# ByteDance-Seed/VeOmni

Hardware: AMD Instinct MI355X
Metric: tokens/sec/node (higher is better)
Workload: dtype bf16; 1 GPU; qwen3-moe-30b FSDP2 bf16 seq4096; model=qwen3-moe-30b, global_batch=8, seq_len=4096, parallelism=dp1

## Files before the change

### include/veomni_hip.h

```cpp
#ifndef VEOMNI_HIP_H
#define VEOMNI_HIP_H

#include <stdint.h>

#ifdef __cplusplus
extern "C" {
#endif

const char* vh_last_error(void);

const char* vh_build_info(void);


int vh_expert_histogram(const int64_t* expert_index, int64_t n,
                        int num_experts, int32_t* out, void* stream);

int vh_moe_scatter_bf16(const uint16_t* x, const int32_t* index, uint16_t* out,
                        int64_t M, int64_t N, int topk, void* stream);

int vh_moe_gather_bf16(const uint16_t* x, const int32_t* index, uint16_t* out,
                       int64_t M, int64_t N, int topk, void* stream);


int vh_group_gemm_nk_bf16(const uint16_t* A, const uint16_t* B, uint16_t* C,
                          const int64_t* cumsum, int G, int64_t N, int64_t K,
                          int64_t total_rows, int trans_b, int accumulate,
                          int activation, void* stream);


int vh_group_gemm_nk8_bf16(const uint16_t* A, const uint16_t* B, uint16_t* C,
                           const int64_t* cumsum, int G, int64_t N, int64_t K,
                           int64_t total_rows, int trans_b, void* stream);

int vh_group_gemm_nk256s_bf16(const uint16_t* A, const uint16_t* B,
                              uint16_t* C, const int64_t* cumsum, int G,
                              int64_t N, int64_t K, int64_t total_rows,
                              void* stream);

int vh_group_gemm_mn8_bf16(const uint16_t* A, const uint16_t* B, uint16_t* C,
                           const int64_t* cumsum, int G, int64_t M, int64_t N,
                           void* stream);

int vh_group_gemm_mn_bf16(const uint16_t* A, const uint16_t* B, uint16_t* C,
                          const int64_t* cumsum, int G, int64_t M, int64_t N,
                          void* stream);

int vh_wtranspose_bf16(const uint16_t* src, uint16_t* dst, int E, int64_t M,
                       int64_t N, void* stream);

int vh_transpose_pad_bf16(const uint16_t* src, uint16_t* dst,
                          const int64_t* cumsum, const int64_t* padded_cumsum,
                          int G, int64_t C, int64_t padded_total, void* stream);

int vh_group_gemm_wg256_bf16(const uint16_t* A, const uint16_t* B, uint16_t* C,
                             const int64_t* padded_cumsum, int G, int64_t M,
                             int64_t N, int64_t PR, void* stream);


int vh_moe_silu_mul_weighted_bf16(const uint16_t* fc1, const uint16_t* w_row,
                                  uint16_t* out, int64_t rows, int64_t I,
                                  int has_w, void* stream);

int vh_moe_silu_mul_weighted_bwd_bf16(const uint16_t* dy, const uint16_t* fc1,
                                      const uint16_t* w_row, uint16_t* dfc1,
                                      float* dw_row, int64_t rows, int64_t I,
                                      int has_w, void* stream);

int vh_moe_silu_mul_clamp_weighted_bf16(const uint16_t* fc1,
                                        const uint16_t* w_row, uint16_t* out,
                                        int64_t rows, int64_t I, int has_w,
                                        float limit, void* stream);

int vh_moe_silu_mul_clamp_weighted_bwd_bf16(const uint16_t* dy,
                                            const uint16_t* fc1,
                                            const uint16_t* w_row,
                                            uint16_t* dfc1, float* dw_row,
                                            int64_t rows, int64_t I, int has_w,
                                            float limit, void* stream);

// ... 71 lines not shown
```

### veomni_amd/csrc/vh_group_gemm.hip

```cpp

#include "vh_common.h"
#include "../../include/veomni_hip.h"

namespace {

constexpr int BM = 128, BN = 128, BK = 64;
constexpr int THREADS = 256;

using bf16frag = __attribute__((ext_vector_type(8))) __bf16;

__device__ __forceinline__ void glds16(const bf16_t* g, bf16_t* l) {
  __builtin_amdgcn_global_load_lds(
      (const __attribute__((address_space(1))) unsigned int*)g,
      (__attribute__((address_space(3))) unsigned int*)l, 16, 0, 0);
}

__device__ __forceinline__ int swz(int row, int colb) {
  return colb ^ ((((row >> 1) ^ (row >> 3)) & 7) << 4);
}

struct KStage {
  const bf16_t* src[4];
  int lds_base[4];

// ... 263 lines not shown

  const int col_in = lane & 15;
  const int row_base_in = (lane >> 4) * 4;
#pragma unroll
  for (int i = 0; i < 4; ++i)
#pragma unroll
    for (int j = 0; j < 4; ++j)
#pragma unroll
      for (int rr = 0; rr < 4; ++rr) {
        int64_t m = (int64_t)bm * BM + wr * 64 + i * 16 + row_base_in + rr;
        int64_t n = (int64_t)bn * BN + wc * 64 + j * 16 + col_in;
        if (m < M && n < N) Cg[m * N + n] = f2bf(acc[i][j][rr]);
      }
}

}

extern "C" int vh_group_gemm_nk_bf16(const uint16_t* A, const uint16_t* B,
                                     uint16_t* C, const int64_t* cumsum, int G,
                                     int64_t N, int64_t K, int64_t total_rows,
                                     int trans_b, int accumulate,
                                     int activation, void* stream) {
  hipStream_t s = reinterpret_cast<hipStream_t>(stream);
  if (!accumulate && activation == 0 && trans_b && K % 64 == 0 && N >= 256 &&
      total_rows >= (int64_t)G * 256 && G <= 4096) {
    return vh_group_gemm_nk256s_bf16(A, B, C, cumsum, G, N, K, total_rows,
                                     stream);
  }
  if (!accumulate && activation == 0 && !trans_b && K % 32 == 0 && K >= 1024 &&
      N >= 1024 && total_rows >= 16 * G * 16) {
    return vh_group_gemm_nk8_bf16(A, B, C, cumsum, G, N, K, total_rows, 0,
                                  stream);
  }
  VH_CHECK(K % BK == 0, "K %% 64 != 0 (K=%lld)", (long long)K);
  VH_CHECK(N % 16 == 0, "N %% 16 != 0 (N=%lld)", (long long)N);
  VH_CHECK(G >= 1, "G < 1");
  int tiles_m = (int)((total_rows + BM - 1) / BM);
  if (tiles_m < 1) tiles_m = 1;
  int tiles_n = (int)((N + BN - 1) / BN);
  dim3 grid(tiles_m * tiles_n, G);
  size_t lds = 65536;

#define VH_DISPATCH(TB, AC, ACT_)                                              \
  hipLaunchKernelGGL((k_group_gemm_nk<TB, AC, ACT_>), grid, dim3(THREADS),     \
                     lds, s, reinterpret_cast<const bf16_t*>(A),               \
                     reinterpret_cast<const bf16_t*>(B),                       \
                     reinterpret_cast<bf16_t*>(C), cumsum, G, N, K, tiles_m,   \
                     tiles_n)

  if (trans_b) {
// ... 33 lines not shown
```

### veomni_amd/csrc/vh_group_gemm8.hip

```cpp

#include "vh_common.h"

namespace {

constexpr int BM8 = 256, BN8 = 256, KSUB = 32;
constexpr int THREADS8 = 512;

using bf16frag = __attribute__((ext_vector_type(8))) __bf16;

__device__ __forceinline__ void glds16(const bf16_t* g, bf16_t* l) {
  __builtin_amdgcn_global_load_lds(
      (const __attribute__((address_space(1))) unsigned int*)g,
      (__attribute__((address_space(3))) unsigned int*)l, 16, 0, 0);
}

__device__ __forceinline__ int swz32(int row, int colb) {
  return colb ^ (((row >> 2) & 3) << 4);
}

__device__ __forceinline__ void raw_barrier() {
  asm volatile("" ::: "memory");
  __builtin_amdgcn_s_barrier();
  asm volatile("" ::: "memory");
}
// ... 414 lines not shown
      int o = base + lane * 16;
      int row = o >> 7;
      int colb = o & 127;
      src[i] = s + row_of(row) * ld_elems + (swz64(row, colb) >> 1);
      lds_base[i] = base;
    }
  }

  __device__ __forceinline__ void stage(bf16_t* tile, int64_t k0) const {
#pragma unroll
    for (int i = 0; i < 4; ++i) glds16(src[i] + k0, tile + (lds_base[i] >> 1));
  }
};

__device__ __forceinline__ bf16frag frag_read64(const bf16_t* tile, int row0,
                                                int ks, int lane) {
  int row = row0 + (lane & 15);
  int colb = (ks * 32 + ((lane >> 4) << 3)) * 2;
  int off_b = row * 128 + swz64(row, colb);
  return *reinterpret_cast<const bf16frag*>(
      reinterpret_cast<const char*>(tile) + off_b);
}


__global__ void k_gg_sched(const int64_t* __restrict__ cumsum, int G,
                           int tiles_n, int* __restrict__ ws) {
  if (threadIdx.x == 0 && blockIdx.x == 0) {
    int total = 0;
    int64_t prev = 0;
    for (int g = 0; g < G; ++g) {
      int64_t m = cumsum[g] - prev;
      prev = cumsum[g];
      ws[1 + g] = total;
      total += (int)((m + BM8 - 1) / BM8) * tiles_n;
    }
    ws[1 + G] = total;
    ws[0] = total;
  }
}

__global__ __launch_bounds__(THREADS8, 2) void k_group_gemm_nk256s(
    const bf16_t* __restrict__ A, const bf16_t* __restrict__ B,
    bf16_t* __restrict__ C, const int64_t* __restrict__ cumsum, int G,
    int64_t N, int64_t K, int tiles_n, const int* __restrict__ ws) {
  extern __shared__ __attribute__((aligned(16))) char smem[];
  bf16_t* sm = reinterpret_cast<bf16_t*>(smem);
  auto ta = [&](int buf) { return sm + buf * 32768; };
  auto tb = [&](int buf) { return sm + 16384 + buf * 32768; };

  const int tid = threadIdx.x;
  const int lane = tid & 63;
  const int wave = tid >> 6;
  const int wr = wave >> 2, wc = wave & 3;

  const int total_tiles = ws[0];
  const int X = blockIdx.x & 7;
  const int slot = blockIdx.x >> 3;
  const int L = (total_tiles + 7) / 8;
  const int t_end = min((X + 1) * L, total_tiles);
  const int nk = (int)(K / BK64);

  for (int t = X * L + slot; t < t_end; t += 32) {
    int lo = 0, hi = G - 1;
    while (lo < hi) {
      int mid = (lo + hi + 1) >> 1;
      if (ws[1 + mid] <= t) lo = mid;
      else hi = mid - 1;
    }
    const int gid = lo;
    const int local = t - ws[1 + gid];
    const int tiles_m_g = (ws[2 + gid] - ws[1 + gid]) / tiles_n;
    const int bm = local % tiles_m_g;
    const int bn = local / tiles_m_g;

    const int64_t row_start = (gid > 0) ? cumsum[gid - 1] : 0;
    const int64_t m_size = cumsum[gid] - row_start;
    const bf16_t* Ag = A + row_start * K;
    const bf16_t* Bg = B + (int64_t)gid * N * K;
    bf16_t* Cg = C + row_start * N;

    KStage64 sa, sb;
    sa.init(Ag, K, [&](int r) -> int64_t {
      int64_t gm = (int64_t)bm * BM8 + r;
      return gm % m_size;
    }, tid);
    sb.init(Bg, K, [&](int r) -> int64_t {
      int64_t gn = (int64_t)bn * BN8 + r;
      return gn % N;
    }, tid);

    f32x4 acc[8][4];
#pragma unroll
    for (int i = 0; i < 8; ++i)
#pragma unroll
      for (int j = 0; j < 4; ++j) acc[i][j] = {0.f, 0.f, 0.f, 0.f};

    sa.stage(ta(0), 0);
    sb.stage(tb(0), 0);
    __syncthreads();
    int cur = 0;
    for (int kt = 0; kt < nk; ++kt) {
      if (kt + 1 < nk) {
        sa.stage(ta(cur ^ 1), (int64_t)(kt + 1) * BK64);
        sb.stage(tb(cur ^ 1), (int64_t)(kt + 1) * BK64);
      }
#pragma unroll
      for (int ks = 0; ks < 2; ++ks) {
        bf16frag af[4], bfr[4];
#pragma unroll
        for (int j = 0; j < 4; ++j) bfr[j] = frag_read64(tb(cur), wc * 64 + j * 16, ks, lane);
#pragma unroll
        for (int i = 0; i < 4; ++i) af[i] = frag_read64(ta(cur), wr * 128 + i * 16, ks, lane);
        __builtin_amdgcn_s_setprio(1);
#pragma unroll
        for (int i = 0; i < 4; ++i)
#pragma unroll
          for (int j = 0; j < 4; ++j)
            acc[i][j] = __builtin_amdgcn_mfma_f32_16x16x32_bf16(af[i], bfr[j], acc[i][j], 0, 0, 0);
        __builtin_amdgcn_s_setprio(0);
#pragma unroll
        for (int i = 0; i < 4; ++i) af[i] = frag_read64(ta(cur), wr * 128 + 64 + i * 16, ks, lane);
        __builtin_amdgcn_s_setprio(1);
#pragma unroll
        for (int i = 0; i < 4; ++i)
#pragma unroll
          for (int j = 0; j < 4; ++j)
            acc[i + 4][j] = __builtin_amdgcn_mfma_f32_16x16x32_bf16(af[i], bfr[j], acc[i + 4][j], 0, 0, 0);
        __builtin_amdgcn_s_setprio(0);
      }
      __syncthreads();
      cur ^= 1;
    }

    const int col_in = lane & 15;
    const int row_base_in = (lane >> 4) * 4;
#pragma unroll
    for (int i = 0; i < 8; ++i)
#pragma unroll
      for (int j = 0; j < 4; ++j)
#pragma unroll
        for (int rr = 0; rr < 4; ++rr) {
          int64_t m = (int64_t)bm * BM8 + wr * 128 + (i & 3) * 16 + (i >> 2) * 64 +
                      row_base_in + rr;
          int64_t n = (int64_t)bn * BN8 + wc * 64 + j * 16 + col_in;
          if (m < m_size && n < N) Cg[m * N + n] = f2bf(acc[i][j][rr]);
        }
  }
}

}

static int* vh_gg_sched_ws = nullptr;
static constexpr int VH_GG_SCHED_MAX_G = 4096;

extern "C" int vh_group_gemm_nk256s_bf16(const uint16_t* A, const uint16_t* B,
                                         uint16_t* C, const int64_t* cumsum,
                                         int G, int64_t N, int64_t K,
                                         int64_t total_rows, void* stream) {
  hipStream_t s = reinterpret_cast<hipStream_t>(stream);
  VH_CHECK(K % BK64 == 0, "K %% 64 != 0");
  VH_CHECK(N % 16 == 0, "N %% 16 != 0");
  VH_CHECK(G <= VH_GG_SCHED_MAX_G, "G > %d", VH_GG_SCHED_MAX_G);
  if (vh_gg_sched_ws == nullptr) {
    VH_HIP(hipMalloc(&vh_gg_sched_ws, (VH_GG_SCHED_MAX_G + 2) * sizeof(int)));
  }
  int tiles_n = (int)((N + BN8 - 1) / BN8);
  hipLaunchKernelGGL(k_gg_sched, dim3(1), dim3(64), 0, s, cumsum, G, tiles_n,
                     vh_gg_sched_ws);
  VH_HIP(hipGetLastError());
  hipLaunchKernelGGL(k_group_gemm_nk256s, dim3(256), dim3(THREADS8), 131072, s,
                     reinterpret_cast<const bf16_t*>(A),
                     reinterpret_cast<const bf16_t*>(B),
                     reinterpret_cast<bf16_t*>(C), cumsum, G, N, K, tiles_n,
                     vh_gg_sched_ws);
  VH_HIP(hipGetLastError());
  return 0;
}


namespace {

__global__ void k_transpose_pad(const bf16_t* __restrict__ src,
                                bf16_t* __restrict__ dst,
                                const int64_t* __restrict__ cumsum,
                                const int64_t* __restrict__ padded_cumsum,
                                int G, int64_t C, int64_t padded_total) {
  __shared__ __attribute__((aligned(16))) bf16_t t2[64][72];

  int64_t chunk = blockIdx.x;
  int64_t col0 = (int64_t)blockIdx.y * 64;
  int64_t p0 = chunk * 64;
  int lo = 0, hi = G;
  while (lo < hi) {
    int mid = (lo + hi) >> 1;
    if (p0 >= padded_cumsum[mid]) lo = mid + 1; else hi = mid;
  }
  int g = lo;
  if (g >= G) return;
  int64_t pstart = (g > 0) ? padded_cumsum[g - 1] : 0;
  int64_t sstart = (g > 0) ? cumsum[g - 1] : 0;
  int64_t kcount = cumsum[g] - sstart;
  int64_t local0 = p0 - pstart;

  const int tid = threadIdx.x;
  for (int r = tid / 8; r < 64; r += 32) {
    int64_t lr = local0 + r;
    const int cpos = (tid % 8) * 8;
    bf16x8 v = {};
    if (lr < kcount && col0 + cpos < C) {
      v = *reinterpret_cast<const bf16x8*>(src + (sstart + lr) * C + col0 + cpos);
    }
    *reinterpret_cast<bf16x8*>(&t2[r][cpos]) = v;
  }
  __syncthreads();
  for (int c = tid / 8; c < 64; c += 32) {
    int rpos = (tid % 8) * 8;
    if (col0 + c < C) {
      bf16x8 v;
#pragma unroll
      for (int j = 0; j < 8; ++j) v.v[j] = t2[rpos + j][c];
      *reinterpret_cast<bf16x8*>(dst + (col0 + c) * padded_total + p0 + rpos) = v;
    }
  }
}

__global__ __launch_bounds__(THREADS8, 2) void k_group_gemm_wg256s(
    const bf16_t* __restrict__ A, const bf16_t* __restrict__ B,
    bf16_t* __restrict__ C, const int64_t* __restrict__ padded_cumsum, int G,
    int64_t M, int64_t N, int64_t PR, int tiles_m, int tiles_n) {
  extern __shared__ __attribute__((aligned(16))) char smem[];
  bf16_t* sm = reinterpret_cast<bf16_t*>(smem);
  auto ta = [&](int buf) { return sm + buf * 32768; };
  auto tb = [&](int buf) { return sm + 16384 + buf * 32768; };

  const int tid = threadIdx.x;
  const int lane = tid & 63;
  const int wave = tid >> 6;
  const int wr = wave >> 2, wc = wave & 3;

  const int tpg = tiles_m * tiles_n;
  const int total = G * tpg;
  const int X = blockIdx.x & 7;
  const int slot = blockIdx.x >> 3;
  const int L = (total + 7) / 8;
  const int t_end = min((X + 1) * L, total);

  for (int t = X * L + slot; t < t_end; t += 32) {
    const int gid = t / tpg;
    const int local = t - gid * tpg;
    const int bm = local % tiles_m;
    const int bn = local / tiles_m;

    const int64_t p_start = (gid > 0) ? padded_cumsum[gid - 1] : 0;
    const int64_t klen = padded_cumsum[gid] - p_start;
    bf16_t* Cg = C + (int64_t)gid * M * N;

    f32x4 acc[8][4];
#pragma unroll
    for (int i = 0; i < 8; ++i)
#pragma unroll
      for (int j = 0; j < 4; ++j) acc[i][j] = {0.f, 0.f, 0.f, 0.f};

    if (klen > 0) {
      const bf16_t* Ag = A + p_start;
      const bf16_t* Bg = B + p_start;
      KStage64 sa, sb;
      sa.init(Ag, PR, [&](int r) -> int64_t {
        int64_t gm = (int64_t)bm * BM8 + r;
        return gm % M;
      }, tid);
      sb.init(Bg, PR, [&](int r) -> int64_t {
        int64_t gn = (int64_t)bn * BN8 + r;
        return gn % N;
      }, tid);

      const int nk = (int)(klen / BK64);
      sa.stage(ta(0), 0);
      sb.stage(tb(0), 0);
      __syncthreads();
      int cur = 0;
      for (int kt = 0; kt < nk; ++kt) {
        if (kt + 1 < nk) {
          sa.stage(ta(cur ^ 1), (int64_t)(kt + 1) * BK64);
          sb.stage(tb(cur ^ 1), (int64_t)(kt + 1) * BK64);
        }
#pragma unroll
        for (int ks = 0; ks < 2; ++ks) {
          bf16frag af[4], bfr[4];
#pragma unroll
          for (int j = 0; j < 4; ++j) bfr[j] = frag_read64(tb(cur), wc * 64 + j * 16, ks, lane);
#pragma unroll
          for (int i = 0; i < 4; ++i) af[i] = frag_read64(ta(cur), wr * 128 + i * 16, ks, lane);
          __builtin_amdgcn_s_setprio(1);
#pragma unroll
          for (int i = 0; i < 4; ++i)
#pragma unroll
            for (int j = 0; j < 4; ++j)
              acc[i][j] = __builtin_amdgcn_mfma_f32_16x16x32_bf16(af[i], bfr[j], acc[i][j], 0, 0, 0);
          __builtin_amdgcn_s_setprio(0);
#pragma unroll
          for (int i = 0; i < 4; ++i) af[i] = frag_read64(ta(cur), wr * 128 + 64 + i * 16, ks, lane);
          __builtin_amdgcn_s_setprio(1);
#pragma unroll
          for (int i = 0; i < 4; ++i)
#pragma unroll
            for (int j = 0; j < 4; ++j)
              acc[i + 4][j] = __builtin_amdgcn_mfma_f32_16x16x32_bf16(af[i], bfr[j], acc[i + 4][j], 0, 0, 0);
          __builtin_amdgcn_s_setprio(0);
        }
        __syncthreads();
        cur ^= 1;
      }
    } else {
    }

    const int col_in = lane & 15;
    const int row_base_in = (lane >> 4) * 4;
#pragma unroll
    for (int i = 0; i < 8; ++i)
#pragma unroll
      for (int j = 0; j < 4; ++j)
#pragma unroll
        for (int rr = 0; rr < 4; ++rr) {
          int64_t m = (int64_t)bm * BM8 + wr * 128 + (i & 3) * 16 + (i >> 2) * 64 +
                      row_base_in + rr;
          int64_t n = (int64_t)bn * BN8 + wc * 64 + j * 16 + col_in;
          if (m < M && n < N) Cg[m * N + n] = f2bf(acc[i][j][rr]);
        }
  }
}

}

extern "C" int vh_transpose_pad_bf16(const uint16_t* src, uint16_t* dst,
                                     const int64_t* cumsum,
                                     const int64_t* padded_cumsum, int G,
                                     int64_t C, int64_t padded_total,
                                     void* stream) {
  hipStream_t s = reinterpret_cast<hipStream_t>(stream);
  VH_CHECK(C % 8 == 0, "C %% 8 != 0");
  VH_CHECK(padded_total % 64 == 0, "padded_total %% 64 != 0");
  dim3 grid((uint32_t)(padded_total / 64), (uint32_t)((C + 63) / 64));
  hipLaunchKernelGGL(k_transpose_pad, grid, dim3(256), 0, s,
                     reinterpret_cast<const bf16_t*>(src),
                     reinterpret_cast<bf16_t*>(dst), cumsum, padded_cumsum, G,
                     C, padded_total);
  VH_HIP(hipGetLastError());
  return 0;
}

extern "C" int vh_group_gemm_wg256_bf16(const uint16_t* A, const uint16_t* B,
                                        uint16_t* C,
                                        const int64_t* padded_cumsum, int G,
                                        int64_t M, int64_t N, int64_t PR,
                                        void* stream) {
  hipStream_t s = reinterpret_cast<hipStream_t>(stream);
  VH_CHECK(PR % 64 == 0, "PR %% 64 != 0");
  int tiles_m = (int)((M + BM8 - 1) / BM8);
  int tiles_n = (int)((N + BN8 - 1) / BN8);
  hipLaunchKernelGGL(k_group_gemm_wg256s, dim3(256), dim3(THREADS8), 131072, s,
                     reinterpret_cast<const bf16_t*>(A),
                     reinterpret_cast<const bf16_t*>(B),
                     reinterpret_cast<bf16_t*>(C), padded_cumsum, G, M, N, PR,
                     tiles_m, tiles_n);
  VH_HIP(hipGetLastError());
  return 0;
}
```

### veomni_amd/ops/hip_lib.py

```python

from __future__ import annotations

import ctypes
import os
from typing import Optional

import torch

_LIB: Optional[ctypes.CDLL] = None

_PKG_DIR = os.path.dirname(os.path.dirname(os.path.abspath(__file__)))
SO_PATH = os.path.join(_PKG_DIR, "libveomni_hip.so")

c_i64 = ctypes.c_int64
c_int = ctypes.c_int
c_f32 = ctypes.c_float
c_p = ctypes.c_void_p


def _sig(lib: ctypes.CDLL, name: str, *argtypes) -> None:
    fn = getattr(lib, name)
    fn.restype = ctypes.c_int
    fn.argtypes = list(argtypes)


def get_lib() -> ctypes.CDLL:
    global _LIB
    if _LIB is not None:
        return _LIB
    if not os.path.exists(SO_PATH):
        raise RuntimeError(
            f"libveomni_hip.so not found at {SO_PATH}. Build it with "
            "`python veomni_amd/csrc/build.py` (or __graft_entry__.build()). "
            "The HIP op path has NO fallback by design."
        )
    lib = ctypes.CDLL(SO_PATH)
    lib.vh_last_error.restype = ctypes.c_char_p
    lib.vh_build_info.restype = ctypes.c_char_p
    _sig(lib, "vh_expert_histogram", c_p, c_i64, c_int, c_p, c_p)
    _sig(lib, "vh_moe_scatter_bf16", c_p, c_p, c_p, c_i64, c_i64, c_int, c_p)
    _sig(lib, "vh_moe_gather_bf16", c_p, c_p, c_p, c_i64, c_i64, c_int, c_p)
    _sig(lib, "vh_group_gemm_nk_bf16", c_p, c_p, c_p, c_p, c_int, c_i64, c_i64,
         c_i64, c_int, c_int, c_int, c_p)
    _sig(lib, "vh_group_gemm_nk8_bf16", c_p, c_p, c_p, c_p, c_int, c_i64, c_i64,
         c_i64, c_int, c_p)
    _sig(lib, "vh_group_gemm_nk256s_bf16", c_p, c_p, c_p, c_p, c_int, c_i64,
         c_i64, c_i64, c_p)
    _sig(lib, "vh_group_gemm_mn_bf16", c_p, c_p, c_p, c_p, c_int, c_i64, c_i64, c_p)
    _sig(lib, "vh_transpose_pad_bf16", c_p, c_p, c_p, c_p, c_int, c_i64, c_i64, c_p)
    _sig(lib, "vh_wtranspose_bf16", c_p, c_p, c_int, c_i64, c_i64, c_p)
    _sig(lib, "vh_group_gemm_wg256_bf16", c_p, c_p, c_p, c_p, c_int, c_i64,
         c_i64, c_i64, c_p)
    _sig(lib, "vh_moe_silu_mul_weighted_bf16", c_p, c_p, c_p, c_i64, c_i64, c_int, c_p)
    _sig(lib, "vh_moe_silu_mul_weighted_bwd_bf16", c_p, c_p, c_p, c_p, c_p,
         c_i64, c_i64, c_int, c_p)
    _sig(lib, "vh_moe_silu_mul_clamp_weighted_bf16", c_p, c_p, c_p, c_i64, c_i64,
         c_int, c_f32, c_p)
    _sig(lib, "vh_moe_silu_mul_clamp_weighted_bwd_bf16", c_p, c_p, c_p, c_p, c_p,
         c_i64, c_i64, c_int, c_f32, c_p)
    _sig(lib, "vh_rmsnorm_fwd_bf16", c_p, c_p, c_p, c_p, c_i64, c_i64, c_f32, c_p)
    _sig(lib, "vh_rmsnorm_bwd_bf16", c_p, c_p, c_p, c_p, c_p, c_p, c_i64, c_i64, c_p)
    _sig(lib, "vh_rope_bf16", c_p, c_p, c_p, c_p, c_p, c_p, c_i64, c_i64, c_i64,
         c_i64, c_i64, c_int, c_p)
    _sig(lib, "vh_silu_mul_bf16", c_p, c_p, c_p, c_i64, c_p)
    _sig(lib, "vh_silu_mul_bwd_bf16", c_p, c_p, c_p, c_p, c_p, c_i64, c_p)
    _sig(lib, "vh_ce_fwd_bf16", c_p, c_p, c_p, c_p, c_i64, c_i64, c_f32, c_i64, c_p)
    _sig(lib, "vh_adamw_bf16", c_p, c_p, c_p, c_p, c_p, c_int, c_i64, c_f32,
         c_f32, c_f32, c_f32, c_f32, c_int, c_p, c_p)
    _sig(lib, "vh_attn_fwd_bf16", c_p, c_p, c_p, c_p, c_p, c_int, c_int, c_int,
         c_i64, c_f32, c_p, c_p)
    _sig(lib, "vh_attn_bwd_pre_bf16", c_p, c_p, c_p, c_p, c_p, c_i64, c_p)
    _sig(lib, "vh_attn_bwd2_bf16", c_p, c_p, c_p, c_p, c_p, c_p, c_p, c_p, c_p,
         c_int, c_int, c_int, c_i64, c_f32, c_p, c_p, c_p)
    _sig(lib, "vh_lbl_fwd", c_p, c_int, c_p, c_i64, c_int, c_int, c_p, c_int, c_p)
# ... 105 lines not shown
        a = torch.nn.functional.pad(a, (0, pad))
        b = torch.nn.functional.pad(b, (0, pad) if trans_b else (0, 0, 0, pad))
        K = K + pad
    accumulate = c is not None
    if c is None:
        c = torch.empty(a.shape[0], N, dtype=a.dtype, device=a.device)
    cs = cumsum.to(torch.int64).contiguous()
    with _prof("group_gemm_nk", 2.0 * a.shape[0] * N * K):
        check(get_lib().vh_group_gemm_nk_bf16(
            dptr(a.contiguous()), dptr(b.contiguous()), dptr(c), dptr(cs), G, N, K,
            a.shape[0], int(trans_b), int(accumulate), activation, cur_stream()),
            "vh_group_gemm_nk")
    return c


def group_gemm_mn(a: torch.Tensor, b: torch.Tensor, cumsum: torch.Tensor,
                  G: int) -> torch.Tensor:
    assert a.dtype == torch.bfloat16 and b.dtype == torch.bfloat16
    rows = a.shape[0]
    M, N = a.shape[1], b.shape[1]
    c = torch.empty(G, M, N, dtype=a.dtype, device=a.device)
    cs = cumsum.to(torch.int64).contiguous()
    if M >= 512 and N >= 512 and rows >= 2048:
        counts = torch.diff(cs, prepend=cs.new_zeros(1))
        pad_cs = ((counts + 63) // 64 * 64).cumsum(0).contiguous()
        PR = rows + 64 * G
        at = torch.empty(M, PR, dtype=a.dtype, device=a.device)
        bt = torch.empty(N, PR, dtype=a.dtype, device=a.device)
        lib = get_lib()
        with _prof("wgrad_transpose", 2.0 * rows * (M + N) * 2):
            check(lib.vh_transpose_pad_bf16(dptr(a.contiguous()), dptr(at), dptr(cs),
                                            dptr(pad_cs), G, M, PR, cur_stream()),
                  "vh_transpose_pad(a)")
            check(lib.vh_transpose_pad_bf16(dptr(b.contiguous()), dptr(bt), dptr(cs),
                                            dptr(pad_cs), G, N, PR, cur_stream()),
                  "vh_transpose_pad(b)")
        with _prof("group_gemm_mn", 2.0 * rows * M * N):
            check(lib.vh_group_gemm_wg256_bf16(dptr(at), dptr(bt), dptr(c),
                                               dptr(pad_cs), G, M, N, PR,
                                               cur_stream()), "vh_group_gemm_wg256")
        return c
    with _prof("group_gemm_mn", 2.0 * rows * M * N):
        check(get_lib().vh_group_gemm_mn_bf16(
            dptr(a.contiguous()), dptr(b.contiguous()), dptr(c), dptr(cs), G, M, N,
            cur_stream()), "vh_group_gemm_mn")
    return c


def weight_transpose(b: torch.Tensor) -> torch.Tensor:
    E, M, N = b.shape
    if M % 64 or N % 64 or b.dtype != torch.bfloat16:
        return b.transpose(1, 2).contiguous()
    out = torch.empty(E, N, M, dtype=b.dtype, device=b.device)
    with _prof("wtranspose", 2.0 * E * M * N * 2):
        check(get_lib().vh_wtranspose_bf16(dptr(b.contiguous()), dptr(out), E,
                                           M, N, cur_stream()), "vh_wtranspose")
    return out


def swiglu_limit_bf16(limit: float) -> float:
    return float(torch.tensor(limit, dtype=torch.bfloat16))


# ... 237 lines not shown
```

### veomni_amd/ops/kernels/moe.py

```python

from __future__ import annotations

import functools
import math

import torch

from ...distributed.moe import dispatch_to_ep_class
from ...distributed.parallel_state import get_parallel_state
from .. import hip_lib
from ..kernel_registry import KERNEL_REGISTRY, HardwareRequirement, KernelSpec

_fused_moe_forward = None


def compute_expert_scatter_index(expert_index: torch.Tensor):
    flat = expert_index.flatten()
    sorted_order = flat.argsort(stable=True)
    inv = torch.empty_like(sorted_order)
    inv[sorted_order] = torch.arange(sorted_order.numel(), dtype=sorted_order.dtype,
                                     device=sorted_order.device)
    return sorted_order, inv.to(torch.int32).view(expert_index.shape)


# ... 14 lines not shown
        scattered_w = torch.empty_like(w)
        scattered_w[scatter_index.flatten().to(torch.int64)] = w
        weighted = hip_lib.silu_mul_weighted(fc1, scattered_w, swiglu_limit)

        fc2 = hip_lib.group_gemm_nk(weighted, fc2_weight, cumsum_t, trans_b=True)
        out = hip_lib.moe_gather(fc2, scatter_index)

        ctx.num_experts = num_experts
        ctx.swiglu_limit = swiglu_limit
        ctx.save_for_backward(gate_weights, fc1_1_2_weight, fc2_weight,
                              scatter_index, scatter_output, cumsum_t, fc1,
                              scattered_w, weighted)
        return out

    @staticmethod
    def backward(ctx, grad_output):
        (gate_weights, fc1_1_2_weight, fc2_weight, scatter_index,
         scatter_output, cumsum_t, fc1, scattered_w, weighted) = ctx.saved_tensors
        G = fc2_weight.shape[0]
        grad_output = grad_output.view(-1, grad_output.shape[-1]).contiguous()

        grad_fc2_out = hip_lib.moe_scatter(grad_output, scatter_index)
        d_weighted = hip_lib.group_gemm_nk(
            grad_fc2_out, hip_lib.weight_transpose(fc2_weight), cumsum_t, trans_b=True)
        d_fc2_w = hip_lib.group_gemm_mn(grad_fc2_out, weighted, cumsum_t, G)

        d_fc1, dw_rows = hip_lib.silu_mul_weighted_bwd(d_weighted, fc1, scattered_w,
                                                       ctx.swiglu_limit)
        grad_gate = dw_rows[scatter_index.flatten().to(torch.int64)]
        grad_gate = grad_gate.reshape(gate_weights.shape).to(gate_weights.dtype)

        d_scatter = hip_lib.group_gemm_nk(
            d_fc1, hip_lib.weight_transpose(fc1_1_2_weight), cumsum_t, trans_b=True)
        d_fc1_w = hip_lib.group_gemm_mn(d_fc1, scatter_output, cumsum_t, G)

        grad_hidden = hip_lib.moe_gather(d_scatter, scatter_index)
        return None, grad_gate, None, grad_hidden, d_fc1_w, d_fc2_w, None


class EPMergedFc1HipGroupGemm(torch.autograd.Function):

    @staticmethod
    def forward(ctx, permute_tokens, cumsum, fc1_1_2_weight, fc2_weight,
                swiglu_limit=None):
        fc1 = hip_lib.group_gemm_nk(permute_tokens, fc1_1_2_weight, cumsum, trans_b=True)
        act = hip_lib.silu_mul_weighted(fc1, None, swiglu_limit)
        fc2 = hip_lib.group_gemm_nk(act, fc2_weight, cumsum, trans_b=True)
        ctx.swiglu_limit = swiglu_limit
        ctx.save_for_backward(permute_tokens, cumsum, fc1_1_2_weight, fc2_weight, fc1, act)
        return fc2

    @staticmethod
    def backward(ctx, grad_output):
        permute_tokens, cumsum, fc1_1_2_weight, fc2_weight, fc1, act = ctx.saved_tensors
        G = fc2_weight.shape[0]
        grad_output = grad_output.contiguous()
        d_act = hip_lib.group_gemm_nk(
            grad_output, hip_lib.weight_transpose(fc2_weight), cumsum, trans_b=True)
        d_fc2_w = hip_lib.group_gemm_mn(grad_output, act, cumsum, G)
        d_fc1, _ = hip_lib.silu_mul_weighted_bwd(d_act, fc1, None, ctx.swiglu_limit)
        d_tokens = hip_lib.group_gemm_nk(
            d_fc1, hip_lib.weight_transpose(fc1_1_2_weight), cumsum, trans_b=True)
        d_fc1_w = hip_lib.group_gemm_mn(d_fc1, permute_tokens, cumsum, G)
        return d_tokens, None, d_fc1_w, d_fc2_w, None



def _ep_mlp_fwd(tokens, cumsum, fc1_1_2_weight, fc2_weight, swiglu_limit=None):
    fc1 = hip_lib.group_gemm_nk(tokens, fc1_1_2_weight, cumsum, trans_b=True)
    act = hip_lib.silu_mul_weighted(fc1, None, swiglu_limit)
    fc2 = hip_lib.group_gemm_nk(act, fc2_weight, cumsum, trans_b=True)
    return fc2, (tokens, fc1_1_2_weight, fc2_weight, fc1, act)


def _ep_mlp_bwd_dgrad(dY, cumsum, saved, swiglu_limit=None):
    _, w1, w2, fc1, _ = saved
    d_act = hip_lib.group_gemm_nk(dY, hip_lib.weight_transpose(w2), cumsum,
                                  trans_b=True)
    d_fc1, _ = hip_lib.silu_mul_weighted_bwd(d_act, fc1, None, swiglu_limit)
    d_tokens = hip_lib.group_gemm_nk(d_fc1, hip_lib.weight_transpose(w1),
                                     cumsum, trans_b=True)
    return d_tokens, (dY, d_fc1)


def _ep_mlp_bwd_wgrad(cumsum, saved, stash):
    tokens, _, w2, _, act = saved
    dY, d_fc1 = stash
    G = w2.shape[0]
    d_fc2_w = hip_lib.group_gemm_mn(dY, act, cumsum, G)
    d_fc1_w = hip_lib.group_gemm_mn(d_fc1, tokens, cumsum, G)
    return (d_fc1_w, d_fc2_w)


def _make_ep_a2a(swiglu_limit=None):
    from ...distributed.moe import make_ep_a2a_class

    if swiglu_limit is None:
        return make_ep_a2a_class(_ep_mlp_fwd, _ep_mlp_bwd_dgrad, _ep_mlp_bwd_wgrad)
    return make_ep_a2a_class(
        functools.partial(_ep_mlp_fwd, swiglu_limit=swiglu_limit),
        functools.partial(_ep_mlp_bwd_dgrad, swiglu_limit=swiglu_limit),
        _ep_mlp_bwd_wgrad)


# ... 99 lines not shown
```

Baseline: 14640 tokens/s.

## Read transposed operands in-kernel with ds_read_tr instead of explicit transpose copies

Adds a K-major B variant of the grouped nk256s GEMM that stages untransposed weight tiles and reads them with LDS transpose loads (ds_read_b64_tr_b16). The MoE backward dgrad calls then pass the weights directly, which removes the weight_transpose copies. The weight-gradient GEMM is also rewritten to read row-major activations straight from global memory, clamping and zero-filling the ragged per-expert tails. This replaces the separate transpose_pad kernels and padded buffers. Both changes remove extra memory passes and allocations, at the cost of more complex LDS addressing and an extra vmcnt wait per iteration.

```diff
diff --git a/include/veomni_hip.h b/include/veomni_hip.h
--- a/include/veomni_hip.h
+++ b/include/veomni_hip.h
@@ -37,6 +37,11 @@
                               int64_t N, int64_t K, int64_t total_rows,
                               void* stream);
 
+int vh_group_gemm_nk256s_kn_bf16(const uint16_t* A, const uint16_t* B,
+                                 uint16_t* C, const int64_t* cumsum, int G,
+                                 int64_t N, int64_t K, int64_t total_rows,
+                                 void* stream);
+
 int vh_group_gemm_mn8_bf16(const uint16_t* A, const uint16_t* B, uint16_t* C,
                            const int64_t* cumsum, int G, int64_t M, int64_t N,
                            void* stream);
@@ -48,13 +53,9 @@
 int vh_wtranspose_bf16(const uint16_t* src, uint16_t* dst, int E, int64_t M,
                        int64_t N, void* stream);
 
-int vh_transpose_pad_bf16(const uint16_t* src, uint16_t* dst,
-                          const int64_t* cumsum, const int64_t* padded_cumsum,
-                          int G, int64_t C, int64_t padded_total, void* stream);
-
-int vh_group_gemm_wg256_bf16(const uint16_t* A, const uint16_t* B, uint16_t* C,
-                             const int64_t* padded_cumsum, int G, int64_t M,
-                             int64_t N, int64_t PR, void* stream);
+int vh_group_gemm_wgd_bf16(const uint16_t* A, const uint16_t* B, uint16_t* C,
+                           const int64_t* cumsum, int G, int64_t M, int64_t N,
+                           int64_t total_rows, void* stream);
 
 
 int vh_moe_silu_mul_weighted_bf16(const uint16_t* fc1, const uint16_t* w_row,
diff --git a/veomni_amd/csrc/vh_group_gemm.hip b/veomni_amd/csrc/vh_group_gemm.hip
--- a/veomni_amd/csrc/vh_group_gemm.hip
+++ b/veomni_amd/csrc/vh_group_gemm.hip
@@ -309,10 +309,13 @@
                                      int trans_b, int accumulate,
                                      int activation, void* stream) {
   hipStream_t s = reinterpret_cast<hipStream_t>(stream);
-  if (!accumulate && activation == 0 && trans_b && K % 64 == 0 && N >= 256 &&
+  if (!accumulate && activation == 0 && K % 64 == 0 && N >= 256 &&
       total_rows >= (int64_t)G * 256 && G <= 4096) {
-    return vh_group_gemm_nk256s_bf16(A, B, C, cumsum, G, N, K, total_rows,
-                                     stream);
+    if (trans_b)
+      return vh_group_gemm_nk256s_bf16(A, B, C, cumsum, G, N, K, total_rows,
+                                       stream);
+    return vh_group_gemm_nk256s_kn_bf16(A, B, C, cumsum, G, N, K, total_rows,
+                                        stream);
   }
   if (!accumulate && activation == 0 && !trans_b && K % 32 == 0 && K >= 1024 &&
       N >= 1024 && total_rows >= 16 * G * 16) {
diff --git a/veomni_amd/csrc/vh_group_gemm8.hip b/veomni_amd/csrc/vh_group_gemm8.hip
--- a/veomni_amd/csrc/vh_group_gemm8.hip
+++ b/veomni_amd/csrc/vh_group_gemm8.hip
@@ -1,5 +1,7 @@
 
 #include "vh_common.h"
+
+#include <type_traits>
 
 namespace {
 
@@ -460,6 +462,85 @@
       reinterpret_cast<const char*>(tile) + off_b);
 }
 
+__device__ __forceinline__ int tswz64(int k) {
+  return (k & 3) | (((k >> 3) & 1) << 2);
+}
+
+struct TStage64 {
+  const bf16_t* src;
+  int64_t ld;
+  int krow;
+  int wave;
+
+  template <typename ColFn>
+  __device__ __forceinline__ void init(const bf16_t* s, int64_t ld_elems,
+                                       ColFn col_of, int tid) {
+    const int lane = tid & 63;
+    wave = __builtin_amdgcn_readfirstlane(tid >> 6);
+    krow = wave * 2 + (lane >> 5);
+    const int pb = (lane & 31) * 16;
+    const int seg = (pb >> 5) ^ tswz64(krow);
+    src = s + col_of(seg * 16) + ((pb & 31) >> 1);
+    ld = ld_elems;
+  }
+
+  template <typename RowFn>
+  __device__ __forceinline__ void stage(bf16_t* tile, int k0, RowFn row_of) const {
+#pragma unroll
+    for (int i = 0; i < 4; ++i)
+      glds16(src + (int64_t)row_of(k0 + i * 16 + krow) * ld,
+             tile + ((i * 8192 + wave * 1024) >> 1));
+  }
+
+  __device__ __forceinline__ void zero_tail(bf16_t* tile, int rem, int lane) const {
+#pragma unroll
+    for (int i = 0; i < 4; ++i)
+#pragma unroll
+      for (int b = 0; b < 2; ++b) {
+        const int k = i * 16 + wave * 2 + b;
+        if (k >= rem)
+          *reinterpret_cast<uint2*>(reinterpret_cast<char*>(tile) + k * 512 +
+                                    lane * 8) = uint2{0u, 0u};
+      }
+  }
+};
+
+using u32x2 = __attribute__((ext_vector_type(2))) uint32_t;
+using u32x4 = __attribute__((ext_vector_type(4))) uint32_t;
+struct TrFrag { u32x2 lo, hi; };
+
+__device__ __forceinline__ uint32_t lds_addr(const void* p) {
+  return (uint32_t)(size_t)(const __attribute__((address_space(3))) char*)p;
+}
+
+__device__ __forceinline__ int tr_lane_off(int out0, int lane) {
+  const int k = ((lane >> 4) << 3) + ((lane >> 2) & 3);
+  return k * 512 + (((out0 >> 4) ^ tswz64(k)) << 5) + (lane & 3) * 8;
+}
+
+template <int KS>
+__device__ __forceinline__ void tr_issue(TrFrag& f, uint32_t addr) {
+  asm volatile(
+      "ds_read_b64_tr_b16 %0, %2 offset:%3\n\t"
+      "ds_read_b64_tr_b16 %1, %2 offset:%4"
+      : "=&v"(f.lo), "=&v"(f.hi)
+      : "v"(addr), "n"(KS * 16384), "n"(KS * 16384 + 2048)
+      : "memory");
+}
+
+__device__ __forceinline__ void tr_wait(TrFrag (&f)[4]) {
+  asm volatile("s_waitcnt lgkmcnt(0)"
+               : "+v"(f[0].lo), "+v"(f[0].hi), "+v"(f[1].lo), "+v"(f[1].hi),
+                 "+v"(f[2].lo), "+v"(f[2].hi), "+v"(f[3].lo), "+v"(f[3].hi)
+               :
+               : "memory");
+}
+
+__device__ __forceinline__ bf16frag tr_frag(const TrFrag& f) {
+  u32x4 u{f.lo.x, f.lo.y, f.hi.x, f.hi.y};
+  return __builtin_bit_cast(bf16frag, u);
+}
+
 
 __global__ void k_gg_sched(const int64_t* __restrict__ cumsum, int G,
                            int tiles_n, int* __restrict__ ws) {
@@ -477,6 +558,7 @@
   }
 }
 
+template <bool BKN>
 __global__ __launch_bounds__(THREADS8, 2) void k_group_gemm_nk256s(
     const bf16_t* __restrict__ A, const bf16_t* __restrict__ B,
     bf16_t* __restrict__ C, const int64_t* __restrict__ cumsum, int G,
@@ -518,14 +600,28 @@
     bf16_t* Cg = C + row_start * N;
 
     KStage64 sa, sb;
+    TStage64 sbt;
     sa.init(Ag, K, [&](int r) -> int64_t {
       int64_t gm = (int64_t)bm * BM8 + r;
       return gm % m_size;
     }, tid);
-    sb.init(Bg, K, [&](int r) -> int64_t {
-      int64_t gn = (int64_t)bn * BN8 + r;
-      return gn % N;
-    }, tid);
+    if constexpr (BKN) {
+      sbt.init(Bg, N, [&](int c) -> int64_t {
+        return ((int64_t)bn * BN8 + c) % N;
+      }, tid);
+    } else {
+      sb.init(Bg, K, [&](int r) -> int64_t {
+        int64_t gn = (int64_t)bn * BN8 + r;
+        return gn % N;
+      }, tid);
+    }
+    auto stage_b = [&](bf16_t* tile, int kt) {
+      if constexpr (BKN) sbt.stage(tile, kt * BK64, [](int k) { return k; });
+      else sb.stage(tile, (int64_t)kt * BK64);
+    };
+    int btr_off[4];
+#pragma unroll
+    for (int j = 0; j < 4; ++j) btr_off[j] = tr_lane_off(wc * 64 + j * 16, lane);
 
     f32x4 acc[8][4];
 #pragma unroll
@@ -534,14 +630,48 @@
       for (int j = 0; j < 4; ++j) acc[i][j] = {0.f, 0.f, 0.f, 0.f};
 
     sa.stage(ta(0), 0);
-    sb.stage(tb(0), 0);
+    stage_b(tb(0), 0);
+    if constexpr (BKN) VMCNT(0);
     __syncthreads();
     int cur = 0;
     for (int kt = 0; kt < nk; ++kt) {
       if (kt + 1 < nk) {
         sa.stage(ta(cur ^ 1), (int64_t)(kt + 1) * BK64);
-        sb.stage(tb(cur ^ 1), (int64_t)(kt + 1) * BK64);
+        stage_b(tb(cur ^ 1), kt + 1);
       }
+      auto ks_step = [&](auto ks_c) {
+        constexpr int ks = decltype(ks_c)::value;
+        bf16frag af[4], bfr[4];
+        TrFrag tf[4];
+        const uint32_t b0 = lds_addr(tb(cur));
+#pragma unroll
+        for (int j = 0; j < 4; ++j) tr_issue<ks>(tf[j], b0 + btr_off[j]);
+#pragma unroll
+        for (int i = 0; i < 4; ++i) af[i] = frag_read64(ta(cur), wr * 128 + i * 16, ks, lane);
+        tr_wait(tf);
+#pragma unroll
+        for (int j = 0; j < 4; ++j) bfr[j] = tr_frag(tf[j]);
+        __builtin_amdgcn_s_setprio(1);
+#pragma unroll
+        for (int i = 0; i < 4; ++i)
+#pragma unroll
+          for (int j = 0; j < 4; ++j)
+            acc[i][j] = __builtin_amdgcn_mfma_f32_16x16x32_bf16(af[i], bfr[j], acc[i][j], 0, 0, 0);
+        __builtin_amdgcn_s_setprio(0);
+#pragma unroll
+        for (int i = 0; i < 4; ++i) af[i] = frag_read64(ta(cur), wr * 128 + 64 + i * 16, ks, lane);
+        __builtin_amdgcn_s_setprio(1);
+#pragma unroll
+        for (int i = 0; i < 4; ++i)
+#pragma unroll
+          for (int j = 0; j < 4; ++j)
+            acc[i + 4][j] = __builtin_amdgcn_mfma_f32_16x16x32_bf16(af[i], bfr[j], acc[i + 4][j], 0, 0, 0);
+        __builtin_amdgcn_s_setprio(0);
+      };
+      if constexpr (BKN) {
+        ks_step(std::integral_constant<int, 0>{});
+        ks_step(std::integral_constant<int, 1>{});
+      } else {
 #pragma unroll
       for (int ks = 0; ks < 2; ++ks) {
         bf16frag af[4], bfr[4];
@@ -566,6 +696,8 @@
             acc[i + 4][j] = __builtin_amdgcn_mfma_f32_16x16x32_bf16(af[i], bfr[j], acc[i + 4][j], 0, 0, 0);
         __builtin_amdgcn_s_setprio(0);
       }
+      }
+      if constexpr (BKN) VMCNT(0);
       __syncthreads();
       cur ^= 1;
     }
@@ -591,10 +723,9 @@
 static int* vh_gg_sched_ws = nullptr;
 static constexpr int VH_GG_SCHED_MAX_G = 4096;
 
-extern "C" int vh_group_gemm_nk256s_bf16(const uint16_t* A, const uint16_t* B,
-                                         uint16_t* C, const int64_t* cumsum,
-                                         int G, int64_t N, int64_t K,
-                                         int64_t total_rows, void* stream) {
+static int vh_launch_nk256s(bool b_kn, const uint16_t* A, const uint16_t* B,
+                            uint16_t* C, const int64_t* cumsum, int G,
+                            int64_t N, int64_t K, void* stream) {
   hipStream_t s = reinterpret_cast<hipStream_t>(stream);
   VH_CHECK(K % BK64 == 0, "K %% 64 != 0");
   VH_CHECK(N % 16 == 0, "N %% 16 != 0");
@@ -606,7 +737,8 @@
   hipLaunchKernelGGL(k_gg_sched, dim3(1), dim3(64), 0, s, cumsum, G, tiles_n,
                      vh_gg_sched_ws);
   VH_HIP(hipGetLastError());
-  hipLaunchKernelGGL(k_group_gemm_nk256s, dim3(256), dim3(THREADS8), 131072, s,
+  auto kern = b_kn ? k_group_gemm_nk256s<true> : k_group_gemm_nk256s<false>;
+  hipLaunchKernelGGL(kern, dim3(256), dim3(THREADS8), 131072, s,
                      reinterpret_cast<const bf16_t*>(A),
                      reinterpret_cast<const bf16_t*>(B),
                      reinterpret_cast<bf16_t*>(C), cumsum, G, N, K, tiles_n,
@@ -615,57 +747,29 @@
   return 0;
 }
 
+extern "C" int vh_group_gemm_nk256s_bf16(const uint16_t* A, const uint16_t* B,
+                                         uint16_t* C, const int64_t* cumsum,
+                                         int G, int64_t N, int64_t K,
+                                         int64_t total_rows, void* stream) {
+  (void)total_rows;
+  return vh_launch_nk256s(false, A, B, C, cumsum, G, N, K, stream);
+}
+
+extern "C" int vh_group_gemm_nk256s_kn_bf16(const uint16_t* A, const uint16_t* B,
+                                            uint16_t* C, const int64_t* cumsum,
+                                            int G, int64_t N, int64_t K,
+                                            int64_t total_rows, void* stream) {
+  (void)total_rows;
+  return vh_launch_nk256s(true, A, B, C, cumsum, G, N, K, stream);
+}
+
 
 namespace {
 
-__global__ void k_transpose_pad(const bf16_t* __restrict__ src,
-                                bf16_t* __restrict__ dst,
-                                const int64_t* __restrict__ cumsum,
-                                const int64_t* __restrict__ padded_cumsum,
-                                int G, int64_t C, int64_t padded_total) {
-  __shared__ __attribute__((aligned(16))) bf16_t t2[64][72];
-
-  int64_t chunk = blockIdx.x;
-  int64_t col0 = (int64_t)blockIdx.y * 64;
-  int64_t p0 = chunk * 64;
-  int lo = 0, hi = G;
-  while (lo < hi) {
-    int mid = (lo + hi) >> 1;
-    if (p0 >= padded_cumsum[mid]) lo = mid + 1; else hi = mid;
-  }
-  int g = lo;
-  if (g >= G) return;
-  int64_t pstart = (g > 0) ? padded_cumsum[g - 1] : 0;
-  int64_t sstart = (g > 0) ? cumsum[g - 1] : 0;
-  int64_t kcount = cumsum[g] - sstart;
-  int64_t local0 = p0 - pstart;
-
-  const int tid = threadIdx.x;
-  for (int r = tid / 8; r < 64; r += 32) {
-    int64_t lr = local0 + r;
-    const int cpos = (tid % 8) * 8;
-    bf16x8 v = {};
-    if (lr < kcount && col0 + cpos < C) {
-      v = *reinterpret_cast<const bf16x8*>(src + (sstart + lr) * C + col0 + cpos);
-    }
-    *reinterpret_cast<bf16x8*>(&t2[r][cpos]) = v;
-  }
-  __syncthreads();
-  for (int c = tid / 8; c < 64; c += 32) {
-    int rpos = (tid % 8) * 8;
-    if (col0 + c < C) {
-      bf16x8 v;
-#pragma unroll
-      for (int j = 0; j < 8; ++j) v.v[j] = t2[rpos + j][c];
-      *reinterpret_cast<bf16x8*>(dst + (col0 + c) * padded_total + p0 + rpos) = v;
-    }
-  }
-}
-
-__global__ __launch_bounds__(THREADS8, 2) void k_group_gemm_wg256s(
+__global__ __launch_bounds__(THREADS8, 2) void k_group_gemm_wgd256s(
     const bf16_t* __restrict__ A, const bf16_t* __restrict__ B,
-    bf16_t* __restrict__ C, const int64_t* __restrict__ padded_cumsum, int G,
-    int64_t M, int64_t N, int64_t PR, int tiles_m, int tiles_n) {
+    bf16_t* __restrict__ C, const int64_t* __restrict__ cumsum, int G,
+    int64_t M, int64_t N, int tiles_m, int tiles_n) {
   extern __shared__ __attribute__((aligned(16))) char smem[];
   bf16_t* sm = reinterpret_cast<bf16_t*>(smem);
   auto ta = [&](int buf) { return sm + buf * 32768; };
@@ -689,8 +793,8 @@
     const int bm = local % tiles_m;
     const int bn = local / tiles_m;
 
-    const int64_t p_start = (gid > 0) ? padded_cumsum[gid - 1] : 0;
-    const int64_t klen = padded_cumsum[gid] - p_start;
+    const int64_t row_start = (gid > 0) ? cumsum[gid - 1] : 0;
+    const int cnt = (int)(cumsum[gid] - row_start);
     bf16_t* Cg = C + (int64_t)gid * M * N;
 
     f32x4 acc[8][4];
@@ -699,36 +803,58 @@
 #pragma unroll
       for (int j = 0; j < 4; ++j) acc[i][j] = {0.f, 0.f, 0.f, 0.f};
 
-    if (klen > 0) {
-      const bf16_t* Ag = A + p_start;
-      const bf16_t* Bg = B + p_start;
-      KStage64 sa, sb;
-      sa.init(Ag, PR, [&](int r) -> int64_t {
-        int64_t gm = (int64_t)bm * BM8 + r;
-        return gm % M;
+    if (cnt > 0) {
+      TStage64 sa, sb;
+      sa.init(A + row_start * M, M, [&](int c) -> int64_t {
+        return ((int64_t)bm * BM8 + c) % M;
       }, tid);
-      sb.init(Bg, PR, [&](int r) -> int64_t {
-        int64_t gn = (int64_t)bn * BN8 + r;
-        return gn % N;
+      sb.init(B + row_start * N, N, [&](int c) -> int64_t {
+        return ((int64_t)bn * BN8 + c) % N;
       }, tid);
-
-      const int nk = (int)(klen / BK64);
-      sa.stage(ta(0), 0);
-      sb.stage(tb(0), 0);
+      auto row_of = [&](int k) { return min(k, cnt - 1); };
+
+      const int nk = (cnt + BK64 - 1) / BK64;
+      const int rem = cnt - (nk - 1) * BK64;
+      auto stage = [&](int buf, int kt) {
+        sa.stage(ta(buf), kt * BK64, row_of);
+        sb.stage(tb(buf), kt * BK64, row_of);
+      };
+      auto zero_tail = [&](int buf) {
+        VMCNT(0);
+        sa.zero_tail(ta(buf), rem, lane);
+        sb.zero_tail(tb(buf), rem, lane);
+      };
+
+      int atr_off[8], btr_off[4];
+#pragma unroll
+      for (int i = 0; i < 8; ++i) atr_off[i] = tr_lane_off(wr * 128 + i * 16, lane);
+#pragma unroll
+      for (int j = 0; j < 4; ++j) btr_off[j] = tr_lane_off(wc * 64 + j * 16, lane);
+
+      stage(0, 0);
+      if (nk == 1 && rem < BK64) zero_tail(0);
+      VMCNT(0);
       __syncthreads();
       int cur = 0;
       for (int kt = 0; kt < nk; ++kt) {
-        if (kt + 1 < nk) {
-          sa.stage(ta(cur ^ 1), (int64_t)(kt + 1) * BK64);
-          sb.stage(tb(cur ^ 1), (int64_t)(kt + 1) * BK64);
-        }
-#pragma unroll
-        for (int ks = 0; ks < 2; ++ks) {
+        if (kt + 1 < nk) stage(cur ^ 1, kt + 1);
+        const uint32_t a0 = lds_addr(ta(cur)), b0 = lds_addr(tb(cur));
+        auto ks_step = [&](auto ks_c) {
+          constexpr int ks = decltype(ks_c)::value;
+          TrFrag tb4[4], ta4[4], ta4h[4];
+#pragma unroll
+          for (int j = 0; j < 4; ++j) tr_issue<ks>(tb4[j], b0 + btr_off[j]);
+#pragma unroll
+          for (int i = 0; i < 4; ++i) tr_issue<ks>(ta4[i], a0 + atr_off[i]);
+          tr_wait(tb4);
+          tr_wait(ta4);
+#pragma unroll
+          for (int i = 0; i < 4; ++i) tr_issue<ks>(ta4h[i], a0 + atr_off[4 + i]);
           bf16frag af[4], bfr[4];
 #pragma unroll
-          for (int j = 0; j < 4; ++j) bfr[j] = frag_read64(tb(cur), wc * 64 + j * 16, ks, lane);
-#pragma unroll
-          for (int i = 0; i < 4; ++i) af[i] = frag_read64(ta(cur), wr * 128 + i * 16, ks, lane);
+          for (int j = 0; j < 4; ++j) bfr[j] = tr_frag(tb4[j]);
+#pragma unroll
+          for (int i = 0; i < 4; ++i) af[i] = tr_frag(ta4[i]);
           __builtin_amdgcn_s_setprio(1);
 #pragma unroll
           for (int i = 0; i < 4; ++i)
@@ -736,8 +862,9 @@
             for (int j = 0; j < 4; ++j)
               acc[i][j] = __builtin_amdgcn_mfma_f32_16x16x32_bf16(af[i], bfr[j], acc[i][j], 0, 0, 0);
           __builtin_amdgcn_s_setprio(0);
-#pragma unroll
-          for (int i = 0; i < 4; ++i) af[i] = frag_read64(ta(cur), wr * 128 + 64 + i * 16, ks, lane);
+          tr_wait(ta4h);
+#pragma unroll
+          for (int i = 0; i < 4; ++i) af[i] = tr_frag(ta4h[i]);
           __builtin_amdgcn_s_setprio(1);
 #pragma unroll
           for (int i = 0; i < 4; ++i)
@@ -745,11 +872,14 @@
             for (int j = 0; j < 4; ++j)
               acc[i + 4][j] = __builtin_amdgcn_mfma_f32_16x16x32_bf16(af[i], bfr[j], acc[i + 4][j], 0, 0, 0);
           __builtin_amdgcn_s_setprio(0);
-        }
+        };
+        ks_step(std::integral_constant<int, 0>{});
+        ks_step(std::integral_constant<int, 1>{});
+        if (kt + 2 == nk && rem < BK64) zero_tail(cur ^ 1);
+        VMCNT(0);
         __syncthreads();
         cur ^= 1;
       }
-    } else {
     }
 
     const int col_in = lane & 15;
@@ -770,37 +900,21 @@
 
 }
 
-extern "C" int vh_transpose_pad_bf16(const uint16_t* src, uint16_t* dst,
-                                     const int64_t* cumsum,
-                                     const int64_t* padded_cumsum, int G,
-                                     int64_t C, int64_t padded_total,
-                                     void* stream) {
+extern "C" int vh_group_gemm_wgd_bf16(const uint16_t* A, const uint16_t* B,
+                                      uint16_t* C, const int64_t* cumsum, int G,
+                                      int64_t M, int64_t N, int64_t total_rows,
+                                      void* stream) {
   hipStream_t s = reinterpret_cast<hipStream_t>(stream);
-  VH_CHECK(C % 8 == 0, "C %% 8 != 0");
-  VH_CHECK(padded_total % 64 == 0, "padded_total %% 64 != 0");
-  dim3 grid((uint32_t)(padded_total / 64), (uint32_t)((C + 63) / 64));
-  hipLaunchKernelGGL(k_transpose_pad, grid, dim3(256), 0, s,
-                     reinterpret_cast<const bf16_t*>(src),
-                     reinterpret_cast<bf16_t*>(dst), cumsum, padded_cumsum, G,
-                     C, padded_total);
+  (void)total_rows;
+  VH_CHECK(M % 16 == 0 && N % 16 == 0, "M/N %% 16 != 0");
+  VH_CHECK(G >= 1, "G < 1");
+  int tiles_m = (int)((M + BM8 - 1) / BM8);
+  int tiles_n = (int)((N + BN8 - 1) / BN8);
+  hipLaunchKernelGGL(k_group_gemm_wgd256s, dim3(256), dim3(THREADS8), 131072, s,
+                     reinterpret_cast<const bf16_t*>(A),
+                     reinterpret_cast<const bf16_t*>(B),
+                     reinterpret_cast<bf16_t*>(C), cumsum, G, M, N, tiles_m,
+                     tiles_n);
   VH_HIP(hipGetLastError());
   return 0;
 }
-
-extern "C" int vh_group_gemm_wg256_bf16(const uint16_t* A, const uint16_t* B,
-                                        uint16_t* C,
-                                        const int64_t* padded_cumsum, int G,
-                                        int64_t M, int64_t N, int64_t PR,
-                                        void* stream) {
-  hipStream_t s = reinterpret_cast<hipStream_t>(stream);
-  VH_CHECK(PR % 64 == 0, "PR %% 64 != 0");
-  int tiles_m = (int)((M + BM8 - 1) / BM8);
-  int tiles_n = (int)((N + BN8 - 1) / BN8);
-  hipLaunchKernelGGL(k_group_gemm_wg256s, dim3(256), dim3(THREADS8), 131072, s,
-                     reinterpret_cast<const bf16_t*>(A),
-                     reinterpret_cast<const bf16_t*>(B),
-                     reinterpret_cast<bf16_t*>(C), padded_cumsum, G, M, N, PR,
-                     tiles_m, tiles_n);
-  VH_HIP(hipGetLastError());
-  return 0;
-}
diff --git a/veomni_amd/ops/hip_lib.py b/veomni_amd/ops/hip_lib.py
--- a/veomni_amd/ops/hip_lib.py
+++ b/veomni_amd/ops/hip_lib.py
@@ -46,10 +46,11 @@
          c_i64, c_int, c_p)
     _sig(lib, "vh_group_gemm_nk256s_bf16", c_p, c_p, c_p, c_p, c_int, c_i64,
          c_i64, c_i64, c_p)
+    _sig(lib, "vh_group_gemm_nk256s_kn_bf16", c_p, c_p, c_p, c_p, c_int, c_i64,
+         c_i64, c_i64, c_p)
     _sig(lib, "vh_group_gemm_mn_bf16", c_p, c_p, c_p, c_p, c_int, c_i64, c_i64, c_p)
-    _sig(lib, "vh_transpose_pad_bf16", c_p, c_p, c_p, c_p, c_int, c_i64, c_i64, c_p)
     _sig(lib, "vh_wtranspose_bf16", c_p, c_p, c_int, c_i64, c_i64, c_p)
-    _sig(lib, "vh_group_gemm_wg256_bf16", c_p, c_p, c_p, c_p, c_int, c_i64,
+    _sig(lib, "vh_group_gemm_wgd_bf16", c_p, c_p, c_p, c_p, c_int, c_i64,
          c_i64, c_i64, c_p)
     _sig(lib, "vh_moe_silu_mul_weighted_bf16", c_p, c_p, c_p, c_i64, c_i64, c_int, c_p)
     _sig(lib, "vh_moe_silu_mul_weighted_bwd_bf16", c_p, c_p, c_p, c_p, c_p,
@@ -201,23 +202,10 @@
     c = torch.empty(G, M, N, dtype=a.dtype, device=a.device)
     cs = cumsum.to(torch.int64).contiguous()
     if M >= 512 and N >= 512 and rows >= 2048:
-        counts = torch.diff(cs, prepend=cs.new_zeros(1))
-        pad_cs = ((counts + 63) // 64 * 64).cumsum(0).contiguous()
-        PR = rows + 64 * G
-        at = torch.empty(M, PR, dtype=a.dtype, device=a.device)
-        bt = torch.empty(N, PR, dtype=a.dtype, device=a.device)
-        lib = get_lib()
-        with _prof("wgrad_transpose", 2.0 * rows * (M + N) * 2):
-            check(lib.vh_transpose_pad_bf16(dptr(a.contiguous()), dptr(at), dptr(cs),
-                                            dptr(pad_cs), G, M, PR, cur_stream()),
-                  "vh_transpose_pad(a)")
-            check(lib.vh_transpose_pad_bf16(dptr(b.contiguous()), dptr(bt), dptr(cs),
-                                            dptr(pad_cs), G, N, PR, cur_stream()),
-                  "vh_transpose_pad(b)")
         with _prof("group_gemm_mn", 2.0 * rows * M * N):
-            check(lib.vh_group_gemm_wg256_bf16(dptr(at), dptr(bt), dptr(c),
-                                               dptr(pad_cs), G, M, N, PR,
-                                               cur_stream()), "vh_group_gemm_wg256")
+            check(get_lib().vh_group_gemm_wgd_bf16(
+                dptr(a.contiguous()), dptr(b.contiguous()), dptr(c), dptr(cs), G,
+                M, N, rows, cur_stream()), "vh_group_gemm_wgd")
         return c
     with _prof("group_gemm_mn", 2.0 * rows * M * N):
         check(get_lib().vh_group_gemm_mn_bf16(
diff --git a/veomni_amd/ops/kernels/moe.py b/veomni_amd/ops/kernels/moe.py
--- a/veomni_amd/ops/kernels/moe.py
+++ b/veomni_amd/ops/kernels/moe.py
@@ -60,7 +60,7 @@
 
         grad_fc2_out = hip_lib.moe_scatter(grad_output, scatter_index)
         d_weighted = hip_lib.group_gemm_nk(
-            grad_fc2_out, hip_lib.weight_transpose(fc2_weight), cumsum_t, trans_b=True)
+            grad_fc2_out, fc2_weight, cumsum_t, trans_b=False)
         d_fc2_w = hip_lib.group_gemm_mn(grad_fc2_out, weighted, cumsum_t, G)
 
         d_fc1, dw_rows = hip_lib.silu_mul_weighted_bwd(d_weighted, fc1, scattered_w,
@@ -69,7 +69,7 @@
         grad_gate = grad_gate.reshape(gate_weights.shape).to(gate_weights.dtype)
 
         d_scatter = hip_lib.group_gemm_nk(
-            d_fc1, hip_lib.weight_transpose(fc1_1_2_weight), cumsum_t, trans_b=True)
+            d_fc1, fc1_1_2_weight, cumsum_t, trans_b=False)
         d_fc1_w = hip_lib.group_gemm_mn(d_fc1, scatter_output, cumsum_t, G)
 
         grad_hidden = hip_lib.moe_gather(d_scatter, scatter_index)
@@ -93,12 +93,10 @@
         permute_tokens, cumsum, fc1_1_2_weight, fc2_weight, fc1, act = ctx.saved_tensors
         G = fc2_weight.shape[0]
         grad_output = grad_output.contiguous()
-        d_act = hip_lib.group_gemm_nk(
-            grad_output, hip_lib.weight_transpose(fc2_weight), cumsum, trans_b=True)
+        d_act = hip_lib.group_gemm_nk(grad_output, fc2_weight, cumsum, trans_b=False)
         d_fc2_w = hip_lib.group_gemm_mn(grad_output, act, cumsum, G)
         d_fc1, _ = hip_lib.silu_mul_weighted_bwd(d_act, fc1, None, ctx.swiglu_limit)
-        d_tokens = hip_lib.group_gemm_nk(
-            d_fc1, hip_lib.weight_transpose(fc1_1_2_weight), cumsum, trans_b=True)
+        d_tokens = hip_lib.group_gemm_nk(d_fc1, fc1_1_2_weight, cumsum, trans_b=False)
         d_fc1_w = hip_lib.group_gemm_mn(d_fc1, permute_tokens, cumsum, G)
         return d_tokens, None, d_fc1_w, d_fc2_w, None
 
@@ -113,11 +111,9 @@
 
 def _ep_mlp_bwd_dgrad(dY, cumsum, saved, swiglu_limit=None):
     _, w1, w2, fc1, _ = saved
-    d_act = hip_lib.group_gemm_nk(dY, hip_lib.weight_transpose(w2), cumsum,
-                                  trans_b=True)
+    d_act = hip_lib.group_gemm_nk(dY, w2, cumsum, trans_b=False)
     d_fc1, _ = hip_lib.silu_mul_weighted_bwd(d_act, fc1, None, swiglu_limit)
-    d_tokens = hip_lib.group_gemm_nk(d_fc1, hip_lib.weight_transpose(w1),
-                                     cumsum, trans_b=True)
+    d_tokens = hip_lib.group_gemm_nk(d_fc1, w1, cumsum, trans_b=False)
     return d_tokens, (dY, d_fc1)
 
 
```

After: 15240 tokens/s (median of 6 runs). +4.1%, better.
